# astrodeepnet/debvader

Hardware: AMD Instinct MI355X
Metric: galaxy stamps/sec (train fwd+bwd+Adam) 59x59x6 (higher is better)
Workload: dtype f32; 1 GPU; BASELINE configs[1]: 6-band 59x59 stamps, batch=256 per GPU, latent_dim=32, filters [32,64,128,256], fp32, stage-1 VAE train step; global_batch=256, per_gpu_batch=256, parallelism=dp1

## Files before the change

debvader_amd/csrc/common.h:

```cpp
#pragma once
#include <hip/hip_runtime.h>
#include <stdint.h>
#include <stddef.h>

namespace dv {

enum : int {
  OK = 0,
  E_INVALID = -1,
  E_HIP = -2,
  E_NOMEM = -3,
  E_RCCL = -4,
  E_STATE = -5,
  E_NODEVICE = -6,
};

void set_error(const char* fmt, ...);
int hip_fail(hipError_t e, const char* what, const char* file, int line);

#define DV_HIP(call)                                                     \
  do {                                                                   \
    hipError_t e__ = (call);                                             \
    if (e__ != hipSuccess) return dv::hip_fail(e__, #call, __FILE__, __LINE__); \
  } while (0)
// ... 128 lines not shown
struct GStripParams {
  const float* X;
  const float* W;
  float* U;
  float* A;
  const float* bias;
  const float* alpha;
  const float* zero;
  int NB, H, Wd, Cin, Cout;
  unsigned long long tapcode, wtcode;
  int epi;
  int R, patch_floats, strips_per_stamp, nstrips, strips_per_wg;
};
int launch_gconv_strip(GStripParams p, bool nmajor, hipStream_t s);
int launch_gconv_strip8(GStripParams p, hipStream_t s);

struct WinoParams {
  const float* X;
  const float* Ut;
  float* U;
  float* A;
  const float* bias;
  const float* alpha;
  const float* zero;
  int NB, H, Cin, Cout;
  int epi;
  int nbh, nct, NC, groups, items, items_per_wg;
};
struct WinoWDesc {
  const float* W;
  float* Ut;
  int Cin, Cout, nmajor;
  int wtmap[9];
};
struct WinoWgradParams {
  const float* X;
  const float* Y;
  float* part;
  size_t part_capacity;
  const float* zero;
  int NB, H, Cx, Cy;
  int nbh, nkt, nnt, nblocks, S, bps;
};
bool wino_wgrad_supported(int NB, int H, int Cx, int Cy);
size_t wino_wgrad_part_floats(int NB, int H, int Cx, int Cy, int* splits_out);
int launch_wino_wgrad(WinoWgradParams p, float* out, hipStream_t s);
int launch_wino_wgrad_finish(const float* part, float* out, int S, int Cx, int Cy, hipStream_t s);
bool wino_supported(int NB, int H, int Cin, int Cout);
size_t wino_weight_floats(int Cin, int Cout);
int launch_wino_weights(const WinoWDesc* descs_dev, const WinoWDesc* descs_host, int n, hipStream_t s);
int launch_wino_conv(WinoParams p, hipStream_t s);

struct GConvS2Params {
  const float* X;
  const float* W;
  float* U;
  float* A;
  const float* bias;
  const float* alpha;
  int NB, Hin, Win, Cin;
  int Hout, Wout, Cout;
  int Hc, Wc, M;
  int epi;
  int ndh[4], ndw[4];
  int cph[4], cpw[4];
  int wt[4][4];
  unsigned* dbg_out;
};
int launch_gconv_s2(const GConvS2Params& p, hipStream_t s);
void debug_set_gconv_s2_tile(int code);
void debug_set_wino_variant(int v);
void debug_set_gconv_s2_dbg(unsigned* out);

struct WGradParams {
  const float* X;
  const float* Y;
  float* part;
  int NB, Hx, Wx, Cx;
  int Hy, Wy, Cy;
  int Hc, Wc, sx, sy, ph, pw;
  int ntaps;
  TapTab xt;
  int P;
  int rows_total;
// ... 163 lines not shown
```

debvader_amd/csrc/engine.hip:

```cpp
#include <rccl/rccl.h>
#include <math.h>
#include <stdarg.h>
#include <stdio.h>
#include <stdlib.h>
#include <string.h>
#include <unistd.h>

#include <algorithm>
#include <string>
#include <thread>
#include <map>
#include <mutex>
#include <set>
#include <vector>
#ifdef DV_DEBUG_EXPORTS
#include <functional>
#endif

#include "../../include/debvader_hip.h"
#ifdef DV_DEBUG_EXPORTS
#include "../../include/debvader_hip_debug.h"
#endif
#include <chrono>
#include "common.h"
// ... 301 lines not shown
namespace dv {
struct InferPipe;
}

struct dv_ctx {
  int device = 0, rank = 0, world = 1;
  hipStream_t stream = nullptr;
  hipStream_t comm_stream = nullptr;
  hipStream_t aux_stream = nullptr;
  hipStream_t red_stream = nullptr;
  hipEvent_t ev_red = nullptr;
  hipStream_t lane_stream[3] = {nullptr, nullptr, nullptr};
  hipEvent_t ev_lane[3] = {nullptr, nullptr, nullptr};
  hipEvent_t ev_ready = nullptr, ev_join = nullptr, ev_buf[3] = {nullptr, nullptr, nullptr};
  hipEvent_t ev_dec = nullptr, ev_enc = nullptr, ev_comm = nullptr, ev_small = nullptr, ev_small2 = nullptr;
  hipEvent_t ev_mid = nullptr;
  hipEvent_t ev_wred = nullptr;
  ncclComm_t comm = nullptr;
  bool cprof_on = false;
  std::vector<std::pair<hipEvent_t, hipEvent_t>> cprof_comm, cprof_wait;
  std::vector<hipEvent_t> cprof_pool;
  bool fake_peers = false;
  float* red_dev = nullptr;
  std::vector<dv_model*> models;
};

struct ProfRec {
  int klass;
  int fam;
  hipEvent_t a, b;
};
enum {
  PF_NONE = -1, PF_GCONV2 = 0, PF_GCONV_S2, PF_GSTRIP, PF_GSTRIP8, PF_GCONV, PF_WGRAD, PF_WSTRIP, PF_BCONV, PF_BWGRAD,
  PF_WINO, PF_WINOW, PF_BTRUNK, PF_COUNT
};
static const char* const kProfFamName[PF_COUNT] = {
    "gconv2_kernel", "gconv_s2_kernel", "gconv_strip_kernel", "gconv_strip8_kernel", "gconv_kernel", "wgrad_kernel",
    "wgrad_strip_kernel / wgrad_strip8_kernel", "bconv_kernel", "bwgrad_kernel", "wino_conv4_kernel / wino_conv_kernel", "wino_wgrad_kernel",
    "bgemm_kernel / bgemm_tn_kernel"};

struct DataSlot {
  float* x = nullptr;
  float* y = nullptr;
  int64_t n = 0;
  bool streamed = false;
  const char *hx = nullptr, *hy = nullptr;
  bool x64 = false, y64 = false;
  int64_t sx = 0, sy = 0;
  int64_t h2d_bytes = 0;
  hipEvent_t ready = nullptr;
};

struct StreamRing {
  static constexpr int kDepth = 4;
  static constexpr int kRel = 4;
  float* dev[kDepth] = {};
  float* host[kDepth] = {};
  size_t yoff = 0;
  hipStream_t copy = nullptr;
  hipEvent_t h2d[kDepth] = {};
  hipEvent_t rel[kDepth][kRel] = {};
  bool queued[kDepth] = {};
  unsigned next = 0;
  int threads = 1;
  std::vector<int32_t> iota;
};

struct BfW {
  void* f = nullptr;
  void* d = nullptr;
  int Kf = 0, Kd = 0;
};
// ... 226 lines not shown
  m->prof_launches[k] -= 1;
  if (fam >= 0) {
    m->fam_launches[fam] -= 1;
    m->fam_flops[fam] -= flops;
    m->fam_exec[fam] -= exec < 0 ? flops : exec;
    m->fam_bytes[fam] -= bytes;
  }
}

static int prof_flush(dv_model* m) {
  prof_close(m);
  if (m->prof.empty()) return OK;
  DV_HIP(hipStreamSynchronize(m->ctx->stream));
  for (auto& r : m->prof) {
    float ms = 0.f;
    DV_HIP(hipEventElapsedTime(&ms, r.a, r.b));
    m->prof_ms[r.klass] += ms;
    if (r.fam >= 0) m->fam_ms[r.fam] += ms;
    m->ev_pool.push_back(r.a);
    m->ev_pool.push_back(r.b);
  }
  for (int k = 0; k < 3; ++k) {
    m->prof_n[k] += m->prof_launches[k];
    m->prof_launches[k] = 0;
  }
  m->prof.clear();
  return OK;
}


static bool g_force_v1 = false;
static bool g_no_special = false;
static bool g_no_wino = false;

static hipEvent_t cprof_event(dv_ctx* c) {
  hipEvent_t e = nullptr;
  if (!c->cprof_pool.empty()) {
    e = c->cprof_pool.back();
    c->cprof_pool.pop_back();
  } else {
    (void)hipEventCreate(&e);
  }
  return e;
}
static int comm_allreduce(dv_ctx* c, float* buf, size_t n) {
  hipEvent_t a = nullptr;
  if (c->cprof_on) {
    a = cprof_event(c);
    DV_HIP(hipEventRecord(a, c->comm_stream));
  }
  DV_NCCL(ncclAllReduce(buf, buf, n, ncclFloat, ncclSum, c->comm, c->comm_stream));
  if (a) {
    hipEvent_t b = cprof_event(c);
    DV_HIP(hipEventRecord(b, c->comm_stream));
    c->cprof_comm.push_back({a, b});
  }
  return OK;
}
static int main_waits_for_comm(dv_ctx* c, hipEvent_t ev) {
  hipEvent_t a = nullptr;
  if (c->cprof_on) {
    a = cprof_event(c);
    DV_HIP(hipEventRecord(a, c->stream));
  }
  DV_HIP(hipStreamWaitEvent(c->stream, ev, 0));
  if (a) {
// ... 96 lines not shown
  if (!m->tiny_call || NB > 16 || q.nclass < 1 || !m->ws4 || m->prof_on || epi > 2) return 0;
  const long M = (long)NB * Hout * Hout;
  const long MN = M * Cout;
  const long tiles64 = ((M + 63) / 64) * (long)((Cout + 63) / 64);
  if (tiles64 > 64 || nchunks < 16 || (MN & 3) || (Cout & 3)) return 0;
  const size_t ws4_cap = m->ws4_elems / 4;
  float* ws4 = m->ws4 + (size_t)m->lane_id * ws4_cap;
  int ks = (int)std::min<long>(std::min<long>(16, nchunks / 4), (long)(ws4_cap / (size_t)MN));
  ks = (int)std::min<long>(ks, std::max<long>(1, 512 / tiles64));
  if (ks < 2) return 0;
  q.ksplit = ks;
  q.U = ws4;
  q.A = nullptr;
  q.epi = 0;
  q.bias = nullptr;
  q.alpha = nullptr;
  {
    ProfScope ps(m, 0, nullptr, PF_GCONV2, flops);
    DV_TRY(launch_gconv2(q, fwd_stream(m)));
  }
  ProfScope ps(m, 2);
  DV_TRY(launch_splitk_finish(ws4, ks, MN, Cout, epi >= 1 ? bias : nullptr, epi == 2 ? alpha : nullptr,
                              (long)Hout * Hout * Cout, U, epi == 2 ? Aout : nullptr, fwd_stream(m)));
  return 1;
}

static WinoEntry* wino_find(dv_model* m, const float* W, bool nmajor, const Taps& tp) {
  int wtmap[9];
  for (int t = 0; t < 9; ++t) {
    const int dh = (int)((tp.tapcode >> (4 * t)) & 3) - 1, dw = (int)((tp.tapcode >> (4 * t + 2)) & 3) - 1;
    wtmap[(dh + 1) * 3 + (dw + 1)] = (int)((tp.wtcode >> (4 * t)) & 15);
  }
  for (auto& e : m->wino)
    if (e.d.W == W && e.d.nmajor == (nmajor ? 1 : 0) && !memcmp(e.d.wtmap, wtmap, sizeof wtmap)) return &e;
  return nullptr;
}
static int wino_register(dv_model* m, const float* W, bool nmajor, const Taps& tp, int Cin, int Cout, WinoEntry** out) {
  WinoEntry e;
  memset(&e.d, 0, sizeof e.d);
  e.d.W = W; e.d.Cin = Cin; e.d.Cout = Cout; e.d.nmajor = nmajor ? 1 : 0;
  for (int t = 0; t < 9; ++t) {
    const int dh = (int)((tp.tapcode >> (4 * t)) & 3) - 1, dw = (int)((tp.tapcode >> (4 * t + 2)) & 3) - 1;
    e.d.wtmap[(dh + 1) * 3 + (dw + 1)] = (int)((tp.wtcode >> (4 * t)) & 15);
  }
  DV_TRY(dalloc(m, &e.d.Ut, wino_weight_floats(Cin, Cout)));
  m->wino.push_back(e);
  if (out) *out = &m->wino.back();
  return OK;
}
static int wino_upload_descs(dv_model* m, hipStream_t st) {
  if (m->wino_descs_cap < m->wino.size()) {
    float* q = nullptr;
    const size_t cap = m->wino.size() + 16;
    DV_TRY(dalloc(m, &q, (cap * sizeof(WinoWDesc) + 3) / 4));
    m->wino_descs_dev = reinterpret_cast<WinoWDesc*>(q);
    m->wino_descs_cap = cap;
  }
  std::vector<WinoWDesc> h(m->wino.size());
  for (size_t i = 0; i < h.size(); ++i) h[i] = m->wino[i].d;
  DV_HIP(hipMemcpyAsync(m->wino_descs_dev, h.data(), h.size() * sizeof(WinoWDesc), hipMemcpyHostToDevice, st));
  DV_HIP(hipStreamSynchronize(st));
  return OK;
}
static int wino_refresh_all(dv_model* m, hipStream_t st) {
  if (m->wino.empty()) return OK;
  bool stale = false;
  for (auto& e : m->wino) stale = stale || e.epoch != m->param_epoch;
  if (!stale) return OK;
// ... 1 lines not shown
  for (size_t i = 0; i < h.size(); ++i) h[i] = m->wino[i].d;
  ProfScope ps(m, 2, st);
  DV_TRY(launch_wino_weights(m->wino_descs_dev, h.data(), (int)h.size(), st));
  for (auto& e : m->wino) e.epoch = m->param_epoch;
  return OK;
}
static int wino_conv(dv_model* m, const float* X, const float* W, bool nmajor, const Taps& tp, const float* bias,
                     const float* alpha, float* U, float* Aout, int epi, int NB, int H, int Cin, int Cout, double flops) {
  if (!m->use_wino || g_no_wino || m->tiny_call || m->bf.on || !m->zero_page || !wino_supported(NB, H, Cin, Cout)) return 1;
  if (Cin < 32 || Cout < 32) return 1;
  WinoEntry* e = wino_find(m, W, nmajor, tp);
  hipStream_t st = fwd_stream(m);
  if (!e) {
    DV_TRY(wino_register(m, W, nmajor, tp, Cin, Cout, &e));
    DV_TRY(wino_upload_descs(m, st));
  }
  if (e->epoch == ~(uint64_t)0) {
    const size_t i = (size_t)(e - m->wino.data());
    ProfScope ps(m, 2, st);
    DV_TRY(launch_wino_weights(m->wino_descs_dev + i, &e->d, 1, st));
    e->epoch = m->param_epoch;
  }
  WinoParams p;
  memset(&p, 0, sizeof p);
  p.X = X; p.Ut = e->d.Ut; p.U = U; p.A = Aout; p.bias = bias; p.alpha = alpha; p.zero = m->zero_page;
  p.NB = NB; p.H = H; p.Cin = Cin; p.Cout = Cout; p.epi = epi;
  const double nbh = (H + 7) / 8, groups = ceil((double)NB * nbh * nbh / 4.0);
  const double exec = 2.0 * groups * 4.0 * 16.0 * 16.0 * (double)Cin * (double)(((Cout + 31) / 32) * 32);
  const double bytes = 4.0 * ((double)NB * H * H * (Cin + (U ? Cout : 0) + (Aout ? Cout : 0)) + 16.0 * Cin * Cout +
                              (epi == 2 ? (double)H * H * Cout : 0.0));
  ProfScope ps(m, 0, nullptr, PF_WINO, flops, exec, bytes);
  const int r = launch_wino_conv(p, st);
  if (r > 0) prof_uncount(m, 0, PF_WINO, flops, exec, bytes);
  return r;
}

static int gconv_fprop(dv_model* m, const float* X, const float* W, bool nmajor, const float* bias, const float* alpha,
                       float* U, float* Aout, int epi, int NB, int Hin, int Cin, int Hout, int Cout, int s, int pb,
                       bool single_tap = false, const FuseBwd* fz = nullptr, bool* fused = nullptr, int ksz = 3) {
  if (fused) *fused = false;
  if (single_tap && Hin == 1 && exp_skip_dense()) return OK;
  GConvParams p;
  memset(&p, 0, sizeof p);
  p.X = X;
  p.W = W;
  p.U = U;
  p.A = Aout;
  p.bias = bias;
  p.alpha = alpha;
  p.NB = NB;
  p.Hin = p.Win = Hin;
  p.Cin = Cin;
  p.Hout = p.Wout = Hout;
  p.Cout = Cout;
  p.Hc = p.Wc = Hout;
  p.sin = s;
  p.sout = 1;
  p.ph = p.pw = 0;
  p.M = NB * Hout * Hout;
  p.w_nmajor = nmajor ? 1 : 0;
  p.epi = epi;
  Taps one;
  one.add(0, 0, 0);
  const Taps tp = single_tap ? one : taps_fprop(pb, ksz);
  const bool k3 = single_tap || ksz == 3;
  const double flops = 2.0 * NB * Hout * Hout * tp.n * (double)(W == m->W1p ? m->A.C : Cin) *
// ... 93 lines not shown

static int gconv_dgrad(dv_model* m, const float* X, const float* W, bool nmajor, const float* bias, const float* alpha,
                       float* U, float* Aout, int epi, int NB, int Hs, int Cs, int Ht, int Ct, int s, int pb,
                       const FuseBwd* fz = nullptr, bool* fused = nullptr, int ksz = 3) {
  if (fused) *fused = false;
  const double flops = 2.0 * NB * Hs * Hs * (double)(ksz * ksz) * (double)(W == m->Whp ? 2 * m->A.C : Cs) * (double)Ct;
  const bool k3 = ksz == 3;
  if (k3 && s == 1 && pb == 1 && Hs == Ht && !g_force_v1 && !g_no_special && !(fz && !m->no_fuse)) {
    const Taps tp = taps_dgrad(1, pb, 0, 0);
    if (tp.n == 9) {
      const int r = wino_conv(m, X, W, nmajor, tp, bias, alpha, U, Aout, epi, NB, Ht, Cs, Ct, flops);
      if (r <= 0) return r;
    }
  }
  if (k3 && s == 1 && (Cs == 32 || (Cs == 16 && Ct == 32)) && (Ct == 16 || Ct == 32) && Hs == Ht && Ht >= 8 && Ht <= 64 && !g_force_v1 && !g_no_special &&
      !(fz && !m->no_fuse)) {
    const Taps tp = taps_dgrad(1, pb, 0, 0);
    if (tp.n == 9) {
      GStripParams g;
      memset(&g, 0, sizeof g);
      g.X = X; g.W = W; g.U = U; g.A = Aout; g.bias = bias; g.alpha = alpha; g.zero = m->zero_page;
      g.NB = NB; g.H = Ht; g.Wd = Ht; g.Cin = Cs; g.Cout = Ct;
      g.tapcode = tp.tapcode; g.wtcode = tp.wtcode; g.epi = epi;
      int r;
      {
        ProfScope ps(m, 0, nullptr, PF_GSTRIP, flops);
        r = launch_gconv_strip(g, nmajor, fwd_stream(m));
        if (r > 0) prof_uncount(m, 0, PF_GSTRIP, flops);
      }
      if (r <= 0) return r;
    }
  }
  const bool tiny_splitk = m->tiny_call && NB <= 16 && !fz;
  if (k3 && s == 2 && Cs % 32 == 0 && Ct % 4 == 0 && nmajor && !g_force_v1 && !g_no_special && !(fz && !m->no_fuse) &&
      !tiny_splitk) {
    GConvS2Params q;
    memset(&q, 0, sizeof q);
    q.X = X; q.W = W; q.U = U; q.A = Aout; q.bias = bias; q.alpha = alpha;
    q.NB = NB; q.Hin = q.Win = Hs; q.Cin = Cs; q.Hout = q.Wout = Ht; q.Cout = Ct;
    q.Hc = q.Wc = (Ht + 1) / 2; q.M = NB * q.Hc * q.Wc; q.epi = epi;
    int two = -1, x = 0, kk[2][2] = {{-1, -1}, {-1, -1}};
    bool ok = true;
    for (int ph = 0; ph < 2; ++ph) {
      int n = 0;
      for (int kh = 0; kh < 3; ++kh) {
        const int nh = ph + pb - kh;
        if (nh & 1) continue;
        const int d = nh / 2;
        ++n;
        if (d == 0) kk[ph][0] = kh; else { kk[ph][1] = kh; x = d; two = ph; }
      }
      if (kk[ph][0] < 0 || n > 2) ok = false;
    }
    if (ok && two >= 0 && kk[1 - two][1] < 0) {
      for (int c = 0; c < 4; ++c) {
        q.cph[c] = (c & 2) ? two : 1 - two;
        q.cpw[c] = (c & 1) ? two : 1 - two;
      }
      for (int e = 0; e < 4; ++e) {
        q.ndh[e] = (e & 2) ? x : 0;
        q.ndw[e] = (e & 1) ? x : 0;
        for (int c = 0; c < 4; ++c)
          if ((e & ~c) == 0) q.wt[e][c] = kk[q.cph[c]][(e & 2) ? 1 : 0] * 3 + kk[q.cpw[c]][(e & 1) ? 1 : 0];
      }
      ProfScope ps(m, 0, nullptr, PF_GCONV_S2, flops);
      return launch_gconv_s2(q, fwd_stream(m));
// ... 2296 lines not shown
  hipStream_t s = ctx->stream;
  if (hipMemsetAsync(m->P, 0, A.n_total * sizeof(float), s) != hipSuccess ||
      hipMemsetAsync(m->G, 0, A.n_total * sizeof(float), s) != hipSuccess ||
      hipMemsetAsync(m->Mm, 0, A.n_total * sizeof(float), s) != hipSuccess ||
      hipMemsetAsync(m->Vv, 0, A.n_total * sizeof(float), s) != hipSuccess ||
      hipMemsetAsync(m->scal, 0, 16 * sizeof(float), s) != hipSuccess ||
      hipMemsetAsync(m->zero_page, 0, 64 * sizeof(float), s) != hipSuccess ||
      hipMemsetAsync(m->bnsums, 0, 2 * DV_BN_MAXC * sizeof(float), s) != hipSuccess)
    return fail(E_HIP);
  if (A.dp != A.d || A.twp != A.tw) {
    if (hipMemsetAsync(m->eps, 0, Bc * A.dp * sizeof(float), s) != hipSuccess ||
        hipMemsetAsync(m->z, 0, Bc * A.dp * sizeof(float), s) != hipSuccess ||
        hipMemsetAsync(m->zstd, 0, Bc * A.dp * sizeof(float), s) != hipSuccess ||
        hipMemsetAsync(m->dec_ain, 0, Bc * A.dp * sizeof(float), s) != hipSuccess ||
        hipMemsetAsync(m->t, 0, Bc * A.twp * sizeof(float), s) != hipSuccess)
      return fail(E_HIP);
  }
  if (bf16) {
    st = bf_alloc(m);
    if (st != OK) return fail(st);
  } else if (m->use_wino) {
    auto reg = [&](const float* W, bool nmajor, const Taps& tp, int cin, int cout) -> int {
      if (!wino_supported(1, 8, cin, cout) || tp.n != 9) return OK;
      return wino_register(m, W, nmajor, tp, cin, cout, nullptr);
    };
    const Taps tf = taps_fprop(1), td = taps_dgrad(1, 1, 0, 0);
    for (int j = 0; j < 2 * A.L && st == OK; ++j) {
      int hin, cin, hout, cout, sd;
      A.enc_layer(j, &hin, &cin, &hout, &cout, &sd);
      if (sd == 1 && j > 0) {
        st = reg(m->P + A.specs[A.enc_k(j)].off, false, tf, cin, cout);
        if (st == OK) st = reg(m->P + A.specs[A.enc_k(j)].off, true, td, cout, cin);
      }
      A.dec_layer(j, &hin, &cin, &hout, &cout, &sd);
      if (sd == 1 && st == OK) {
        st = reg(m->P + A.specs[A.dec_k(j)].off, true, td, cin, cout);
        if (st == OK) st = reg(m->P + A.specs[A.dec_k(j)].off, false, tf, cout, cin);
      }
    }
    if (st == OK) st = reg(m->Whp, false, tf, cfg->filters[0], A.C2p);
    if (st == OK) st = reg(m->Whp, true, td, A.C2p, cfg->filters[0]);
    if (st == OK && !m->wino.empty()) st = wino_upload_descs(m, ctx->stream);
    if (st != OK) return fail(st);
  }
  st = dv_model_init(m, 0);
  if (st != OK) return fail(st);
  *out = m;
  return DV_OK;
}

static void philox_host(uint32_t c0, uint32_t c1, uint32_t k0, uint32_t k1, uint32_t out[4]) {
  uint32_t c[4] = {c0, c1, 0x243F6A88u, 0x85A308D3u};
  for (int r = 0; r < 10; ++r) {
    uint64_t p0 = 0xD2511F53ull * c[0], p1 = 0xCD9E8D57ull * c[2];
    uint32_t n0 = (uint32_t)(p1 >> 32) ^ c[1] ^ k0, n1 = (uint32_t)p1;
    uint32_t n2 = (uint32_t)(p0 >> 32) ^ c[3] ^ k1, n3 = (uint32_t)p0;
    c[0] = n0; c[1] = n1; c[2] = n2; c[3] = n3;
    k0 += 0x9E3779B9u;
    k1 += 0xBB67AE85u;
  }
  for (int i = 0; i < 4; ++i) out[i] = c[i];
}

int dv_model_init(dv_model* m, uint64_t seed) {
  if (!m) return DV_E_INVALID;
  const Arch& A = m->A;
  DV_HIP(hipSetDevice(m->ctx->device));
  std::vector<float> h(A.n_total, 0.f);
  for (size_t i = 0; i < A.specs.size(); ++i) {
    const Spec& s = A.specs[i];
    const std::string& n = s.name;
// ... 971 lines not shown
  const size_t nx = (size_t)NB * H * H * Cx, ny = (size_t)NB * H * H * Cy, nw = (size_t)9 * Cx * Cy;
  DV_TRY(debug_buffers(ctx, nx, ny, 2 * nw, &X, &Yb, &out));
  m.ws1_elems = (size_t)16 << 20;
  DV_HIP(hipMalloc((void**)&m.ws1, m.ws1_elems * sizeof(float)));
  DV_HIP(hipMalloc((void**)&m.zero_page, 256));
  DV_HIP(hipMemset(m.zero_page, 0, 256));
  DV_HIP(hipDeviceSynchronize());
  int st = OK;
  for (int pass = 0; pass < 2 && st == OK; ++pass) {
    g_no_wino = pass == 1;
    m.wino_wcount = 0;
    st = wgrad(&m, X, H, Cx, Yb, H, Cy, NB, 1, 1, false, out + pass * nw, Cx, Cx, nullptr);
  }
  g_no_wino = false;
  DV_HIP(hipStreamSynchronize(ctx->stream));
  if (st == OK) {
    std::vector<float> a(nw), b(nw);
    DV_HIP(hipMemcpy(a.data(), out, nw * sizeof(float), hipMemcpyDeviceToHost));
    DV_HIP(hipMemcpy(b.data(), out + nw, nw * sizeof(float), hipMemcpyDeviceToHost));
    double md = 0, mr = 0;
    for (size_t i = 0; i < nw; ++i) {
      md = std::max(md, (double)fabsf(a[i] - b[i]));
      mr = std::max(mr, (double)fabsf(b[i]));
    }
    out2[0] = (float)md;
    out2[1] = (float)mr;
  }
  (void)hipFree(X); (void)hipFree(Yb); (void)hipFree(out); (void)hipFree(m.ws1); (void)hipFree(m.zero_page);
  for (void* q : m.allocs) (void)hipFree(q);
  return st;
}

int dv_debug_winograd(int32_t on) {
  g_no_wino = on == 0;
  if (on >= 1) debug_set_wino_variant(on == 3 ? 1 : 2);
  return DV_OK;
}

int dv_debug_fuse_prelu_bwd(int32_t on) {
  g_fuse_prelu_bwd = on != 0;
  return DV_OK;
}

int dv_debug_general_kernels(int32_t on) {
  g_no_special = on != 0;
  return DV_OK;
}

int dv_debug_mfma_peak(dv_ctx* ctx, int32_t blocks, int32_t iters, int32_t nacc, int32_t randomize, float* out3) {
  if (!ctx || !out3) return DV_E_INVALID;
  DV_HIP(hipSetDevice(ctx->device));
  float* out;
  DV_HIP(hipMalloc((void**)&out, ((size_t)blocks * 256 + 16) * sizeof(float)));
  hipEvent_t a, b;
  DV_HIP(hipEventCreate(&a));
  DV_HIP(hipEventCreate(&b));
  if (nacc != 36) nacc = 16;
  DV_TRY(debug_mfma_peak(out, blocks, iters, nacc, randomize, ctx->stream));
  DV_HIP(hipEventRecord(a, ctx->stream));
  DV_TRY(debug_mfma_peak(out, blocks, iters, nacc, randomize, ctx->stream));
  DV_HIP(hipEventRecord(b, ctx->stream));
  DV_HIP(hipEventSynchronize(b));
  float ms = 0;
  DV_HIP(hipEventElapsedTime(&ms, a, b));
  float h[2];
  DV_HIP(hipMemcpy(h, out, sizeof h, hipMemcpyDeviceToHost));
  out3[0] = (float)((double)blocks * 4 * iters * nacc * 2048.0 / (ms * 1e-3) / 1e12);
// ... 178 lines not shown
```

debvader_amd/csrc/wino.hip:

```cpp
#include "common.h"
#include <algorithm>
#include <type_traits>
#include <stdlib.h>
#include <stdio.h>

namespace dv {

typedef const __attribute__((address_space(1))) void* wn_gptr_t;
typedef __attribute__((address_space(3))) void* wn_lptr_t;

namespace {
constexpr int WN_MB = 4;
constexpr int WN_WAVES = 8;
constexpr int WN_THREADS = 64 * WN_WAVES;
constexpr int WN_PATCH_PIECES = 7;
constexpr int WN_PATCH_FLOATS = WN_PATCH_PIECES * 256;
constexpr int WN_UCH_FLOATS = 16 * 32 * 16;
constexpr int WN_LDS_STAGE = 20;
}

__global__ __launch_bounds__(WN_THREADS, 2) void wino_conv_kernel(const WinoParams p) {
  extern __shared__ __attribute__((aligned(16))) float smem[];
  float* patch = smem;
  float* uch = smem + 2 * WN_MB * WN_PATCH_FLOATS;
// ... 563 lines not shown
              const f32x4 al = *reinterpret_cast<const f32x4*>(alp + px * 32 + nh * 16 + f4 * 4);
              f32x4 o;
#pragma unroll
              for (int e = 0; e < 4; ++e) o[e] = v[e] > 0.f ? v[e] : al[e] * v[e];
              *reinterpret_cast<f32x4*>(p.A + obase + e_aoff[i] + nh * 16) = o;
            }
          }
          __builtin_amdgcn_wave_barrier();
        }
      }
    }
    if (++c == NC) { c = 0; ++it; }
  }
}

__global__ __launch_bounds__(256) void wino_weights_kernel(const WinoWDesc* __restrict__ descs) {
  const WinoWDesc d = descs[blockIdx.y];
  const int NC = d.Cin / 16, nct = (d.Cout + 31) / 32;
  const long total = (long)nct * NC * 512;
  for (long e = (long)blockIdx.x * 256 + threadIdx.x; e < total; e += (long)gridDim.x * 256) {
    const int kk = (int)(e & 15), nn = (int)((e >> 4) & 31);
    const long blk = e >> 9;
    const int kc = (int)(blk % NC), ct = (int)(blk / NC);
    const int k = kc * 16 + kk, n = ct * 32 + nn;
    float g[3][3];
#pragma unroll
    for (int r = 0; r < 3; ++r)
#pragma unroll
      for (int s = 0; s < 3; ++s) {
        const int wt = d.wtmap[r * 3 + s];
        g[r][s] = n < d.Cout ? (d.nmajor ? d.W[((size_t)wt * d.Cout + n) * d.Cin + k] : d.W[((size_t)wt * d.Cin + k) * d.Cout + n])
                             : 0.f;
      }
    float t[4][3];
#pragma unroll
    for (int s = 0; s < 3; ++s) {
      t[0][s] = g[0][s];
      t[1][s] = 0.5f * (g[0][s] + g[1][s] + g[2][s]);
      t[2][s] = 0.5f * (g[0][s] - g[1][s] + g[2][s]);
      t[3][s] = g[2][s];
    }
    float* out = d.Ut + (size_t)blk * (16 * 512) + nn * 16 + ((((kk >> 2) ^ ((0x78 >> (2 * ((nn >> 2) & 3))) & 3)) << 2) | (kk & 3));
#pragma unroll
    for (int i = 0; i < 4; ++i) {
      out[(i * 4 + 0) * 512] = t[i][0];
      out[(i * 4 + 1) * 512] = 0.5f * (t[i][0] + t[i][1] + t[i][2]);
      out[(i * 4 + 2) * 512] = 0.5f * (t[i][0] - t[i][1] + t[i][2]);
      out[(i * 4 + 3) * 512] = t[i][2];
    }
  }
}

namespace {
constexpr int WG_XP = 25;
constexpr int WG_YP = 16;
constexpr int WG_STAGE = (WG_XP + WG_YP) * 256;
}

__global__ __launch_bounds__(256, 1) void wino_wgrad_kernel(const WinoWgradParams p) {
  extern __shared__ __attribute__((aligned(16))) float smem[];
  const int tid = threadIdx.x, lane = tid & 63;
  const int wave = __builtin_amdgcn_readfirstlane(tid >> 6);
  const int l15 = lane & 15, lg = lane >> 4;
  const int H = p.H, Cx = p.Cx, Cy = p.Cy;
  const int nb2 = p.nbh * p.nbh;
  const int tile = blockIdx.x / p.S, split = blockIdx.x - tile * p.S;
  const int kt = tile / p.nnt, nt = tile - kt * p.nnt;
  const int b_begin = split * p.bps, b_end = min(p.nblocks, b_begin + p.bps);
  const int kw = wave >> 1, nw = wave & 1;

  constexpr int NPW = 11;
  unsigned doff[NPW];
  int drc[NPW];
#pragma unroll
  for (int i = 0; i < NPW; ++i) {
// ... 324 lines not shown
```

Baseline: 55540 stamps/s.

## Add Winograd kernel for stride-2 transposed 3x3 convolutions in decoder/backward

Adds a new Winograd-style kernel for stride-2 3x3 convolution paths (transposed/upsampling geometry), with a matching weight transform form and per-geometry tap mapping. Eligible layers (channels >= 64 whose padded tile count pays off) are routed to it before the existing gconv_s2 path. The aim is to cut MFMA work and memory traffic relative to the direct strided-conv kernel. It adds a large new kernel, extra transformed-weight storage, and geometry logic that could mis-handle edge padding.

```diff
diff --git a/debvader_amd/csrc/common.h b/debvader_amd/csrc/common.h
--- a/debvader_amd/csrc/common.h
+++ b/debvader_amd/csrc/common.h
@@ -184,6 +184,7 @@
   float* Ut;
   int Cin, Cout, nmajor;
   int wtmap[9];
+  int form;
 };
 struct WinoWgradParams {
   const float* X;
@@ -202,6 +203,30 @@
 size_t wino_weight_floats(int Cin, int Cout);
 int launch_wino_weights(const WinoWDesc* descs_dev, const WinoWDesc* descs_host, int n, hipStream_t s);
 int launch_wino_conv(WinoParams p, hipStream_t s);
+
+struct WinoS2Params {
+  const float* X;
+  const float* Ut;
+  float* U;
+  float* A;
+  const float* bias;
+  const float* alpha;
+  const float* zero;
+  int NB, Hs, Ht, Cin, Cout;
+  int epi;
+  int da;
+  int j3;
+  int uocode;
+  int nbh, nct, NC, groups, items, items_per_wg;
+};
+struct WinoS2Geo {
+  int two;
+  int da, j3, uocode;
+  int ktap[3];
+};
+bool wino_s2_geometry(int pb, WinoS2Geo* g);
+bool wino_s2_supported(int NB, int Hs, int Ht, int Cin, int Cout);
+int launch_wino_s2(WinoS2Params p, hipStream_t s);
 
 struct GConvS2Params {
   const float* X;
diff --git a/debvader_amd/csrc/engine.hip b/debvader_amd/csrc/engine.hip
--- a/debvader_amd/csrc/engine.hip
+++ b/debvader_amd/csrc/engine.hip
@@ -357,12 +357,12 @@
 };
 enum {
   PF_NONE = -1, PF_GCONV2 = 0, PF_GCONV_S2, PF_GSTRIP, PF_GSTRIP8, PF_GCONV, PF_WGRAD, PF_WSTRIP, PF_BCONV, PF_BWGRAD,
-  PF_WINO, PF_WINOW, PF_BTRUNK, PF_COUNT
+  PF_WINO, PF_WINOW, PF_BTRUNK, PF_WINO_S2, PF_COUNT
 };
 static const char* const kProfFamName[PF_COUNT] = {
     "gconv2_kernel", "gconv_s2_kernel", "gconv_strip_kernel", "gconv_strip8_kernel", "gconv_kernel", "wgrad_kernel",
     "wgrad_strip_kernel / wgrad_strip8_kernel", "bconv_kernel", "bwgrad_kernel", "wino_conv4_kernel / wino_conv_kernel", "wino_wgrad_kernel",
-    "bgemm_kernel / bgemm_tn_kernel"};
+    "bgemm_kernel / bgemm_tn_kernel", "wino_conv_s2t_kernel"};
 
 struct DataSlot {
   float* x = nullptr;
@@ -655,6 +655,7 @@
 static bool g_force_v1 = false;
 static bool g_no_special = false;
 static bool g_no_wino = false;
+static bool g_no_wino_s2 = false;
 
 static hipEvent_t cprof_event(dv_ctx* c) {
   hipEvent_t e = nullptr;
@@ -817,8 +818,27 @@
     wtmap[(dh + 1) * 3 + (dw + 1)] = (int)((tp.wtcode >> (4 * t)) & 15);
   }
   for (auto& e : m->wino)
-    if (e.d.W == W && e.d.nmajor == (nmajor ? 1 : 0) && !memcmp(e.d.wtmap, wtmap, sizeof wtmap)) return &e;
+    if (e.d.form == 0 && e.d.W == W && e.d.nmajor == (nmajor ? 1 : 0) && !memcmp(e.d.wtmap, wtmap, sizeof wtmap)) return &e;
   return nullptr;
+}
+static WinoEntry* wino_s2_find(dv_model* m, const float* W, bool nmajor, const int (&wtmap)[9]) {
+  for (auto& e : m->wino)
+    if (e.d.form == 1 && e.d.W == W && e.d.nmajor == (nmajor ? 1 : 0) && !memcmp(e.d.wtmap, wtmap, sizeof wtmap)) return &e;
+  return nullptr;
+}
+static void wino_s2_wtmap(const WinoS2Geo& g, int (&wtmap)[9]) {
+  for (int a = 0; a < 3; ++a)
+    for (int b = 0; b < 3; ++b) wtmap[a * 3 + b] = g.ktap[a] * 3 + g.ktap[b];
+}
+static int wino_s2_register(dv_model* m, const float* W, bool nmajor, const WinoS2Geo& g, int Cin, int Cout, WinoEntry** out) {
+  WinoEntry e;
+  memset(&e.d, 0, sizeof e.d);
+  e.d.W = W; e.d.Cin = Cin; e.d.Cout = Cout; e.d.nmajor = nmajor ? 1 : 0; e.d.form = 1;
+  wino_s2_wtmap(g, e.d.wtmap);
+  DV_TRY(dalloc(m, &e.d.Ut, wino_weight_floats(Cin, Cout)));
+  m->wino.push_back(e);
+  if (out) *out = &m->wino.back();
+  return OK;
 }
 static int wino_register(dv_model* m, const float* W, bool nmajor, const Taps& tp, int Cin, int Cout, WinoEntry** out) {
   WinoEntry e;
@@ -886,6 +906,44 @@
   ProfScope ps(m, 0, nullptr, PF_WINO, flops, exec, bytes);
   const int r = launch_wino_conv(p, st);
   if (r > 0) prof_uncount(m, 0, PF_WINO, flops, exec, bytes);
+  return r;
+}
+
+static bool wino_s2_takes(int Cs, int Ct, int Ht) {
+  const long hc = (Ht + 1) / 2, hp = (hc + 7) / 8 * 8;
+  return Cs >= 64 && Ct >= 64 && 25 * hp * hp < 36 * hc * hc;
+}
+static int wino_s2_conv(dv_model* m, const float* X, const float* W, bool nmajor, const float* bias, const float* alpha,
+                        float* U, float* Aout, int epi, int NB, int Hs, int Cs, int Ht, int Ct, int pb, double flops) {
+  if (!m->use_wino || g_no_wino || g_no_wino_s2 || m->tiny_call || m->bf.on || !m->zero_page) return 1;
+  WinoS2Geo geo;
+  if (!wino_s2_takes(Cs, Ct, Ht) || !wino_s2_supported(NB, Hs, Ht, Cs, Ct) || !wino_s2_geometry(pb, &geo)) return 1;
+  int wtmap[9];
+  wino_s2_wtmap(geo, wtmap);
+  WinoEntry* e = wino_s2_find(m, W, nmajor, wtmap);
+  hipStream_t st = fwd_stream(m);
+  if (!e) {
+    DV_TRY(wino_s2_register(m, W, nmajor, geo, Cs, Ct, &e));
+    DV_TRY(wino_upload_descs(m, st));
+  }
+  if (e->epoch == ~(uint64_t)0) {
+    const size_t i = (size_t)(e - m->wino.data());
+    ProfScope ps(m, 2, st);
+    DV_TRY(launch_wino_weights(m->wino_descs_dev + i, &e->d, 1, st));
+    e->epoch = m->param_epoch;
+  }
+  WinoS2Params p;
+  memset(&p, 0, sizeof p);
+  p.X = X; p.Ut = e->d.Ut; p.U = U; p.A = Aout; p.bias = bias; p.alpha = alpha; p.zero = m->zero_page;
+  p.NB = NB; p.Hs = Hs; p.Ht = Ht; p.Cin = Cs; p.Cout = Ct; p.epi = epi;
+  p.da = geo.da; p.j3 = geo.j3; p.uocode = geo.uocode;
+  const double nbh = ((Ht + 1) / 2 + 7) / 8, groups = ceil((double)NB * nbh * nbh / 4.0);
+  const double exec = 2.0 * groups * 4.0 * 16.0 * 25.0 * (double)Cs * (double)(((Ct + 31) / 32) * 32);
+  const double bytes = 4.0 * ((double)NB * ((double)Hs * Hs * Cs + (double)Ht * Ht * ((U ? Ct : 0) + (Aout ? Ct : 0))) +
+                              16.0 * Cs * Ct + (epi == 2 ? (double)Ht * Ht * Ct : 0.0));
+  ProfScope ps(m, 0, nullptr, PF_WINO_S2, flops, exec, bytes);
+  const int r = launch_wino_s2(p, st);
+  if (r > 0) prof_uncount(m, 0, PF_WINO_S2, flops, exec, bytes);
   return r;
 }
 
@@ -1045,6 +1103,10 @@
     }
   }
   const bool tiny_splitk = m->tiny_call && NB <= 16 && !fz;
+  if (k3 && s == 2 && !g_force_v1 && !g_no_special && !(fz && !m->no_fuse) && !tiny_splitk) {
+    const int r = wino_s2_conv(m, X, W, nmajor, bias, alpha, U, Aout, epi, NB, Hs, Cs, Ht, Ct, pb, flops);
+    if (r <= 0) return r;
+  }
   if (k3 && s == 2 && Cs % 32 == 0 && Ct % 4 == 0 && nmajor && !g_force_v1 && !g_no_special && !(fz && !m->no_fuse) &&
       !tiny_splitk) {
     GConvS2Params q;
@@ -3407,11 +3469,18 @@
         st = reg(m->P + A.specs[A.enc_k(j)].off, false, tf, cin, cout);
         if (st == OK) st = reg(m->P + A.specs[A.enc_k(j)].off, true, td, cout, cin);
       }
+      WinoS2Geo geo;
+      if (sd == 2 && j > 0 && A.enc_ksz(j) == 3 && wino_s2_takes(cout, cin, hin) && wino_s2_supported(1, hout, hin, cout, cin) &&
+          wino_s2_geometry(same_pad_before(hin, 3, 2, nullptr), &geo))
+        st = wino_s2_register(m, m->P + A.specs[A.enc_k(j)].off, true, geo, cout, cin, nullptr);
       A.dec_layer(j, &hin, &cin, &hout, &cout, &sd);
       if (sd == 1 && st == OK) {
         st = reg(m->P + A.specs[A.dec_k(j)].off, true, td, cin, cout);
         if (st == OK) st = reg(m->P + A.specs[A.dec_k(j)].off, false, tf, cout, cin);
       }
+      if (sd == 2 && st == OK && A.dec_ksz(j) == 3 && wino_s2_takes(cin, cout, hout) && wino_s2_supported(1, hin, hout, cin, cout) &&
+          wino_s2_geometry(same_pad_before(hout, 3, 2, nullptr), &geo))
+        st = wino_s2_register(m, m->P + A.specs[A.dec_k(j)].off, true, geo, cin, cout, nullptr);
     }
     if (st == OK) st = reg(m->Whp, false, tf, cfg->filters[0], A.C2p);
     if (st == OK) st = reg(m->Whp, true, td, A.C2p, cfg->filters[0]);
@@ -4449,7 +4518,15 @@
 }
 
 int dv_debug_winograd(int32_t on) {
+  if (on < 0) {
+    const int q = -on, pb = q & 3, Ht = (q >> 2) & 0xfff, Cs = ((q >> 14) & 0xff) * 16, Ct = ((q >> 22) & 0xff) * 16;
+    WinoS2Geo g;
+    if (!wino_s2_geometry(pb, &g)) return DV_E_INVALID;
+    return (wino_s2_takes(Cs, Ct, Ht) ? 1 : 0) | (g.two << 1) | ((g.da < 0 ? 1 : 0) << 2) | ((g.j3 == 2 ? 1 : 0) << 3) |
+           (g.uocode << 4) | (g.ktap[0] << 12) | (g.ktap[1] << 14) | (g.ktap[2] << 16);
+  }
   g_no_wino = on == 0;
+  g_no_wino_s2 = on == 4;
   if (on >= 1) debug_set_wino_variant(on == 3 ? 1 : 2);
   return DV_OK;
 }
diff --git a/debvader_amd/csrc/wino.hip b/debvader_amd/csrc/wino.hip
--- a/debvader_amd/csrc/wino.hip
+++ b/debvader_amd/csrc/wino.hip
@@ -619,6 +619,25 @@
         g[r][s] = n < d.Cout ? (d.nmajor ? d.W[((size_t)wt * d.Cout + n) * d.Cin + k] : d.W[((size_t)wt * d.Cin + k) * d.Cout + n])
                              : 0.f;
       }
+    float* out = d.Ut + (size_t)blk * (16 * 512) + nn * 16 + ((((kk >> 2) ^ ((0x78 >> (2 * ((nn >> 2) & 3))) & 3)) << 2) | (kk & 3));
+    if (d.form == 1) {
+      float t[4][3];
+#pragma unroll
+      for (int s = 0; s < 3; ++s) {
+        t[0][s] = g[0][s];
+        t[1][s] = g[0][s] + g[1][s];
+        t[2][s] = g[1][s];
+        t[3][s] = g[2][s];
+      }
+#pragma unroll
+      for (int i = 0; i < 4; ++i) {
+        out[(i * 4 + 0) * 512] = t[i][0];
+        out[(i * 4 + 1) * 512] = t[i][0] + t[i][1];
+        out[(i * 4 + 2) * 512] = t[i][1];
+        out[(i * 4 + 3) * 512] = t[i][2];
+      }
+      continue;
+    }
     float t[4][3];
 #pragma unroll
     for (int s = 0; s < 3; ++s) {
@@ -627,7 +646,6 @@
       t[2][s] = 0.5f * (g[0][s] - g[1][s] + g[2][s]);
       t[3][s] = g[2][s];
     }
-    float* out = d.Ut + (size_t)blk * (16 * 512) + nn * 16 + ((((kk >> 2) ^ ((0x78 >> (2 * ((nn >> 2) & 3))) & 3)) << 2) | (kk & 3));
 #pragma unroll
     for (int i = 0; i < 4; ++i) {
       out[(i * 4 + 0) * 512] = t[i][0];
diff --git a/debvader_amd/csrc/wino_s2.hip b/debvader_amd/csrc/wino_s2.hip
--- /dev/null
+++ b/debvader_amd/csrc/wino_s2.hip
@@ -0,0 +1,298 @@
+#include "common.h"
+#include <algorithm>
+#include <stdlib.h>
+
+namespace dv {
+
+typedef const __attribute__((address_space(1))) void* ws_gptr_t;
+typedef __attribute__((address_space(3))) void* ws_lptr_t;
+
+namespace {
+constexpr int S2_MB = 4;
+constexpr int S2_WAVES = 8;
+constexpr int S2_THREADS = 64 * S2_WAVES;
+constexpr int S2_PATCH_PIECES = 6;
+constexpr int S2_PATCH_FLOATS = S2_PATCH_PIECES * 256;
+constexpr int S2_UCH_FLOATS = 16 * 32 * 16;
+constexpr int S2_LDS_STAGE = 20;
+__host__ __device__ constexpr int s2_in(int p) { return p == 0 ? 0 : p == 1 ? 1 : p == 2 ? 2 : p == 3 ? 1 : 3; }
+__host__ __device__ constexpr int s2_w(int p) { return p < 4 ? p : 3; }
+}
+
+__global__ __launch_bounds__(S2_THREADS, 2) void wino_conv_s2t_kernel(const WinoS2Params p) {
+  extern __shared__ __attribute__((aligned(16))) float smem[];
+  float* patch = smem;
+  float* uch = smem + 2 * S2_MB * S2_PATCH_FLOATS;
+  float* stage = uch + 2 * S2_UCH_FLOATS;
+
+  const int tid = threadIdx.x, lane = tid & 63;
+  const int wave = __builtin_amdgcn_readfirstlane(tid >> 6);
+  const int mb = wave & 3, nh = wave >> 2;
+  const int l15 = lane & 15, lg = lane >> 4;
+  const int Hs = p.Hs, Ht = p.Ht, Cin = p.Cin, Cout = p.Cout, NC = p.NC;
+  const int nb2 = p.nbh * p.nbh;
+  const int da = p.da;
+
+  constexpr int NPP = 3;
+  const int k0 = nh * NPP;
+  int prow[NPP], pcol[NPP], prel[NPP];
+#pragma unroll
+  for (int k = 0; k < NPP; ++k) {
+    const int e = 64 * (k0 + k) + lane;
+    const int L = e >> 2;
+    const int pr = L / 9, pc = L - pr * 9;
+    const int q = (e & 3) ^ (pr & 3);
+    prow[k] = L < 81 ? pr + da : -100000;
+    pcol[k] = pc + da;
+    prel[k] = ((pr + da) * Hs + (pc + da)) * Cin + q * 4;
+  }
+
+  const int item0 = blockIdx.x * p.items_per_wg;
+  const int nitems = min(p.items, item0 + p.items_per_wg) - item0;
+  if (nitems <= 0) return;
+  const int qtotal = nitems * NC;
+
+  const float* dm_base = p.zero;
+  const float* dm_usrc = p.zero;
+  float *dm_dstp = patch, *dm_dstu = uch;
+  bool dm_live = false;
+  int dm_by = 0, dm_bx = 0;
+  auto dma_setup = [&](int q, int b) {
+    const int it = q / NC, c = q - it * NC;
+    const int item = item0 + it;
+    const int ct = item / p.groups, g = item - ct * p.groups;
+    const int mblock = g * S2_MB + mb;
+    dm_live = mblock < p.NB * nb2;
+    const int n = dm_live ? mblock / nb2 : 0;
+    const int rem = dm_live ? mblock - n * nb2 : 0;
+    dm_by = rem / p.nbh;
+    dm_bx = rem - dm_by * p.nbh;
+    dm_base = p.X + ((long)(n * Hs + dm_by * 8) * Hs + dm_bx * 8) * Cin + c * 16;
+    dm_dstp = patch + (b * S2_MB + mb) * S2_PATCH_FLOATS + k0 * 256;
+    dm_usrc = p.Ut + ((size_t)(ct * NC + c) * S2_UCH_FLOATS) + wave * 1024 + lane * 4;
+    dm_dstu = uch + b * S2_UCH_FLOATS + wave * 1024;
+  };
+  auto dma_piece = [&](int k) {
+    if (k < NPP) {
+      const bool ok = dm_live && (unsigned)(dm_by * 8 + prow[k]) < (unsigned)Hs && (unsigned)(dm_bx * 8 + pcol[k]) < (unsigned)Hs;
+      const float* src = ok ? dm_base + prel[k] : p.zero;
+      __builtin_amdgcn_global_load_lds((ws_gptr_t)src, (ws_lptr_t)(dm_dstp + k * 256), 16, 0, 0);
+    } else {
+      __builtin_amdgcn_global_load_lds((ws_gptr_t)(dm_usrc + (k - NPP) * 256), (ws_lptr_t)(dm_dstu + (k - NPP) * 256), 16, 0, 0);
+    }
+  };
+
+  const int ty = l15 >> 2, tx = l15 & 3;
+  const int j3 = p.j3;
+  int a_off[4];
+#pragma unroll
+  for (int i = 0; i < 4; ++i) {
+    const int r = 2 * ty + (i < 3 ? i : j3);
+    a_off[i] = (r * 9 + 2 * tx) * 16 + ((lg ^ (r & 3)) << 2);
+  }
+  const int b_off = (nh * 16 + l15) * 16 + ((lg ^ ((0x78 >> (2 * ((l15 >> 2) & 3))) & 3)) << 2);
+  float* stg = stage + wave * (32 * S2_LDS_STAGE);
+
+  auto sync_point = [&]() {
+    asm volatile("s_waitcnt vmcnt(0) lgkmcnt(0)" ::: "memory");
+    __builtin_amdgcn_s_barrier();
+    asm volatile("" ::: "memory");
+  };
+  f32x4 acc[25];
+  dma_setup(0, 0);
+#pragma unroll
+  for (int k = 0; k < NPP + 4; ++k) dma_piece(k);
+  int buf = 0;
+  for (int q = 0; q < qtotal; ++q) {
+    const int it = q / NC, c = q - it * NC;
+    sync_point();
+    const bool more = q + 1 < qtotal;
+    if (more) dma_setup(q + 1, buf ^ 1);
+    if (c == 0) {
+#pragma unroll
+      for (int i = 0; i < 25; ++i) acc[i] = (f32x4){0.f, 0.f, 0.f, 0.f};
+    }
+    const float* P = patch + (buf * S2_MB + mb) * S2_PATCH_FLOATS;
+    const float* Uc = uch + buf * S2_UCH_FLOATS + b_off;
+    f32x4 bfr[16];
+#pragma unroll
+    for (int m = 0; m < 8; ++m) bfr[m] = *reinterpret_cast<const f32x4*>(Uc + (m * 32) * 16);
+    f32x4 V[16];
+    {
+      f32x4 d[4][4];
+#pragma unroll
+      for (int i = 0; i < 4; ++i) {
+#pragma unroll
+        for (int j = 0; j < 3; ++j) d[i][j] = *reinterpret_cast<const f32x4*>(P + a_off[i] + j * 16);
+        d[i][3] = *reinterpret_cast<const f32x4*>(P + a_off[i] + j3 * 16);
+      }
+      __builtin_amdgcn_sched_barrier(0);
+      f32x4 t[4][4];
+#pragma unroll
+      for (int j = 0; j < 4; ++j) {
+        t[0][j] = d[0][j] - d[1][j];
+        t[1][j] = d[1][j];
+        t[2][j] = d[1][j] - d[2][j];
+        t[3][j] = d[3][j];
+      }
+#pragma unroll
+      for (int i = 0; i < 4; ++i) {
+        V[i * 4 + 0] = t[i][0] - t[i][1];
+        V[i * 4 + 1] = t[i][1];
+        V[i * 4 + 2] = t[i][1] - t[i][2];
+        V[i * 4 + 3] = t[i][3];
+      }
+    }
+#pragma unroll
+    for (int g = 0; g < 13; ++g) {
+      const int pa = 2 * g, pbn = 2 * g + 1;
+      if (g == 1) {
+        __builtin_amdgcn_sched_barrier(0);
+#pragma unroll
+        for (int m = 8; m < 16; ++m) bfr[m] = *reinterpret_cast<const f32x4*>(Uc + (m * 32) * 16);
+        __builtin_amdgcn_sched_barrier(0);
+      }
+#pragma unroll
+      for (int jj = 0; jj < 4; ++jj) {
+        {
+          const int vi = s2_in(pa / 5) * 4 + s2_in(pa % 5), wi = s2_w(pa / 5) * 4 + s2_w(pa % 5);
+          acc[pa] = __builtin_amdgcn_mfma_f32_16x16x4f32(V[vi][jj], bfr[wi][jj], acc[pa], 0, 0, 0);
+        }
+        if (pbn < 25) {
+          const int vi = s2_in(pbn / 5) * 4 + s2_in(pbn % 5), wi = s2_w(pbn / 5) * 4 + s2_w(pbn % 5);
+          acc[pbn] = __builtin_amdgcn_mfma_f32_16x16x4f32(V[vi][jj], bfr[wi][jj], acc[pbn], 0, 0, 0);
+        }
+      }
+      if (more && g < 7) {
+        __builtin_amdgcn_sched_barrier(0);
+        dma_piece(g);
+        __builtin_amdgcn_sched_barrier(0);
+      }
+    }
+    if (c == NC - 1) {
+      const int item = item0 + it;
+      const int ct = item / p.groups, g = item - ct * p.groups;
+      const int mblock = g * S2_MB + mb;
+      const bool e_live = mblock < p.NB * nb2;
+      const int e_n = e_live ? mblock / nb2 : 0;
+      const int rem = e_live ? mblock - e_n * nb2 : 0;
+      const int e_by = rem / p.nbh, e_bx = rem - e_by * p.nbh;
+      const int e_col0 = ct * 32 + nh * 16;
+      if (e_live && e_col0 < Cout) {
+        const int f4 = lane & 3;
+        const int e_col = e_col0 + f4 * 4;
+        f32x4 bias4 = {0.f, 0.f, 0.f, 0.f};
+        if (p.epi >= 1) bias4 = *reinterpret_cast<const f32x4*>(p.bias + e_col);
+        const size_t obase = (size_t)e_n * Ht * Ht * Cout;
+#pragma unroll
+        for (int vy = 0; vy < 4; ++vy) {
+          f32x4 tt[5];
+#pragma unroll
+          for (int qc = 0; qc < 5; ++qc) {
+            if (vy == 0) tt[qc] = acc[0 + qc] + acc[5 + qc];
+            else if (vy == 1) tt[qc] = acc[5 + qc] - acc[10 + qc];
+            else if (vy == 2) tt[qc] = acc[15 + qc];
+            else tt[qc] = acc[20 + qc];
+          }
+          const f32x4 y[4] = {tt[0] + tt[1], tt[1] - tt[2], tt[3], tt[4]};
+          const int uy = (p.uocode >> (2 * vy)) & 3;
+#pragma unroll
+          for (int vxh = 0; vxh < 2; ++vxh) {
+#pragma unroll
+            for (int r = 0; r < 4; ++r) {
+              stg[(lg * 8 + 2 * r) * S2_LDS_STAGE + l15] = y[2 * vxh][r];
+              stg[(lg * 8 + 2 * r + 1) * S2_LDS_STAGE + l15] = y[2 * vxh + 1][r];
+            }
+            __builtin_amdgcn_s_waitcnt(0xC07F);
+            __builtin_amdgcn_wave_barrier();
+#pragma unroll
+            for (int k = 0; k < 2; ++k) {
+              const int sidx = k * 16 + (lane >> 2);
+              const int ux = (p.uocode >> (2 * (2 * vxh + (sidx & 1)))) & 3;
+              const int row = e_by * 16 + 4 * (sidx >> 3) + uy, cl = e_bx * 16 + 4 * ((sidx >> 1) & 3) + ux;
+              if (row >= Ht || cl >= Ht) continue;
+              const unsigned aoff = (unsigned)((row * Ht + cl) * Cout + e_col);
+              f32x4 v = *reinterpret_cast<const f32x4*>(stg + sidx * S2_LDS_STAGE + f4 * 4);
+              v += bias4;
+              if (p.U) *reinterpret_cast<f32x4*>(p.U + obase + aoff) = v;
+              if (p.epi == 2) {
+                const f32x4 al = *reinterpret_cast<const f32x4*>(p.alpha + aoff);
+                f32x4 o;
+#pragma unroll
+                for (int e = 0; e < 4; ++e) o[e] = v[e] > 0.f ? v[e] : al[e] * v[e];
+                *reinterpret_cast<f32x4*>(p.A + obase + aoff) = o;
+              }
+            }
+            __builtin_amdgcn_wave_barrier();
+          }
+        }
+      }
+    }
+    buf ^= 1;
+  }
+}
+
+bool wino_s2_geometry(int pb, WinoS2Geo* g) {
+  int two = -1, x = 0, kk[2][2] = {{-1, -1}, {-1, -1}};
+  for (int ph = 0; ph < 2; ++ph) {
+    int n = 0;
+    for (int kh = 0; kh < 3; ++kh) {
+      const int nh = ph + pb - kh;
+      if (nh & 1) continue;
+      const int d = nh / 2;
+      ++n;
+      if (d == 0) kk[ph][0] = kh; else { kk[ph][1] = kh; x = d; two = ph; }
+    }
+    if (kk[ph][0] < 0 || n > 2) return false;
+  }
+  if (two < 0 || kk[1 - two][1] >= 0 || kk[two][1] < 0 || (x != 1 && x != -1)) return false;
+  g->two = two;
+  g->da = x < 0 ? -1 : 0;
+  g->j3 = x < 0 ? 2 : 0;
+  g->ktap[0] = x < 0 ? kk[two][1] : kk[two][0];
+  g->ktap[1] = x < 0 ? kk[two][0] : kk[two][1];
+  g->ktap[2] = kk[1 - two][0];
+  const int u[4] = {two, 2 + two, 2 * (g->da + 1) + (1 - two), 2 * (-g->da) + (1 - two)};
+  g->uocode = u[0] | (u[1] << 2) | (u[2] << 4) | (u[3] << 6);
+  return true;
+}
+
+bool wino_s2_supported(int NB, int Hs, int Ht, int Cin, int Cout) {
+  return Cin >= 16 && Cin % 16 == 0 && Cout >= 16 && Cout % 16 == 0 && Hs >= 2 && Ht >= 2 && Ht <= 2048 && Hs <= 2048 && NB >= 1 &&
+         (size_t)NB * Hs * Hs * (size_t)Cin < ((size_t)1 << 30) && (size_t)Ht * Ht * (size_t)Cout < ((size_t)1 << 30);
+}
+
+int launch_wino_s2(WinoS2Params p, hipStream_t s) {
+  if (!wino_s2_supported(p.NB, p.Hs, p.Ht, p.Cin, p.Cout) || !p.zero || !p.Ut || p.epi < 0 || p.epi > 2) return 1;
+  if (p.epi == 2 && (!p.alpha || !p.A)) return 1;
+  if (p.epi >= 1 && !p.bias) return 1;
+  if ((p.da != 0 && p.da != -1) || (p.j3 != 0 && p.j3 != 2)) return 1;
+  const int Hc = (p.Ht + 1) / 2;
+  p.nbh = (Hc + 7) / 8;
+  p.nct = (p.Cout + 31) / 32;
+  p.NC = p.Cin / 16;
+  const long blocks = (long)p.NB * p.nbh * p.nbh;
+  p.groups = (int)((blocks + S2_MB - 1) / S2_MB);
+  p.items = p.groups * p.nct;
+  static int cus = 0;
+  if (!cus) {
+    int dev = 0;
+    hipDeviceProp_t prop;
+    if (hipGetDevice(&dev) != hipSuccess || hipGetDeviceProperties(&prop, dev) != hipSuccess) return 1;
+    cus = prop.multiProcessorCount > 0 ? prop.multiProcessorCount : 256;
+  }
+  p.items_per_wg = (p.items + cus - 1) / cus;
+  const int grid = (p.items + p.items_per_wg - 1) / p.items_per_wg;
+  const size_t smem = ((size_t)2 * S2_MB * S2_PATCH_FLOATS + 2 * S2_UCH_FLOATS + (size_t)S2_WAVES * 32 * S2_LDS_STAGE) * sizeof(float);
+  static bool attr_set = false;
+  if (!attr_set) {
+    DV_HIP(hipFuncSetAttribute(reinterpret_cast<const void*>(wino_conv_s2t_kernel), hipFuncAttributeMaxDynamicSharedMemorySize,
+                               (int)smem));
+    attr_set = true;
+  }
+  hipLaunchKernelGGL(wino_conv_s2t_kernel, dim3(grid), dim3(S2_THREADS), smem, s, p);
+  DV_HIP(hipGetLastError());
+  return OK;
+}
+
+}
```

Result: no change. 55330 stamps/s, median of 2 (-0.4%).
